# lukebeddow/gripper-mujoco

Measured on AMD Instinct MI355X. Metric: env-steps/sec (batched rollout) at 4096 envs; obs max-rel-err vs C++ ref, higher is better.
Workload: dtype f64; 1 GPU; C3: set6_synthetic 20 mixed objects, randomised spawn (object drawn per episode, spawn_into_scene grid search on the device), steady state: envs staggered over episode steps 1..250 by an untimed pre-roll, benchmark mix (1 episode in 4: the closed-loop grasp-lift-hold program; otherwise the scripted grasp mix: close / squeeze / palm / lift + jitter), canonical sensor/reward config, device auto-rese; envs_per_gpu=4096, global_envs=4096, parallelism=env-shard x1, substeps_per_env_step=63

## Files before the change

__graft_entry__.py:

```python
from __future__ import annotations

import os
import subprocess
import sys

REPO = os.path.dirname(os.path.abspath(__file__))
PKG = os.path.join(REPO, "gripper-mujoco_amd")


def build() -> None:
    if PKG not in sys.path:
        sys.path.insert(0, PKG)
    import threading
    from gmx.build import build as build_lib, build_no_decoupled
    failed = []

    def build_ab():
        try:
            build_no_decoupled()
        except Exception as e:
            failed.append(e)

    ab = threading.Thread(target=build_ab)
    ab.start()
    build_lib(verbose=True)
    ab.join()
    if failed:
        raise failed[0]
    subprocess.run(["make", "-s", "-C", os.path.join(REPO, "oracle"), os.path.join(REPO, "oracle", "liboracle.so")],
                   check=True)
    if os.path.isdir("/root/reference/src"):
        subprocess.run(["make", "-s", "-C", os.path.join(REPO, "oracle"), "ref"], check=True)
    import gmx
    gmx.load_library()


def smoke() -> None:
    import numpy as np
    if PKG not in sys.path:
        sys.path.insert(0, PKG)
    sys.path.insert(0, os.path.join(REPO, "tests"))
    import torch
    assert torch.cuda.is_available(), "smoke() needs a GPU"
    import gmx
    import oracle_lib
    s = gmx.canonical_settings(noise=False, seed=5)
    env = gmx.BatchedGripperEnv(2, object_set="set1_synthetic", settings=s, seed=5, device=0)
    sp = env.make_spawn(x=[0.06, 0.07], y=[0.06, 0.07], idx=0)
    obs0 = env.reset(spawn=sp)
    orc = []
    for e in range(2):
        o = oracle_lib.OracleEnv(env.model, env.cfg, env.objects, e)
        o.reset(sp[e])
        orc.append(o)
        assert np.allclose(obs0[e], o.observation(), atol=1e-5), "reset observation differs from oracle"
    rng = np.random.default_rng(1234)
    for t in range(3):
        a = rng.uniform(-1, 1, size=(2, env.n_actions)).astype(np.float32)
        obs, rew, term, trunc = env.step(a)
        for e in range(2):
            ro, rr, rd = orc[e].step(a[e])
            ro = np.asarray(ro, dtype=np.float64)
            d = np.abs(obs[e] - ro)
            big = np.abs(ro) >= 1e-3
            rel = float((d[big] / np.abs(ro[big])).max()) if big.any() else 0.0
            assert rel <= 1e-4 and float(d[~big].max(initial=0)) <= 1e-4, \
                f"step {t} env {e}: obs rel err {rel:.3e} vs oracle"
            assert bool(term[e]) == bool(rd), "done flag differs from oracle"
            assert abs(float(rew[e]) - float(rr)) <= 1e-5 + 1e-4 * abs(float(rr)), "reward differs from oracle"
    env.close()
    print("smoke ok: 2 envs x 3 env-steps match the oracle")


if __name__ == "__main__":
    build()
    if len(sys.argv) > 1 and sys.argv[1] == "smoke":
        smoke()
```

gripper-mujoco_amd/csrc/gm_capi.hip:

```cpp
#include <hip/hip_runtime.h>

#include <algorithm>
#include <cstddef>
#include <cstdlib>
#include <cstdio>
#include <cmath>
#include <cstring>
#include <map>
#include <string>
#include <vector>
#include <mutex>

#include "gm_kernels.hip"
#include "gm_env_kernels.hip"
#include "gm_policy.hip"
#include "gm_replay.hip"
#include "gm_learn.hip"
#include "gm_ac.hip"
#include "gm_ppo_learn.hip"
#include "gm_sac.hip"
#include "gm_sac_learn.hip"

hipError_t gm_cal_launch_step(int n_seg, int n_envs, hipStream_t st, GmEnvState* states, const gm_model* m,
                              const gm_config* C, const GmTopo* T);
// ... 81 lines not shown

namespace {

int fail(gm_ctx* c, int code, const std::string& msg) {
  if (c) c->err = msg;
  return code;
}
#define HIPCHK(ctx, x)                                                               \
  do {                                                                               \
    hipError_t e_ = (x);                                                             \
    if (e_ != hipSuccess)                                                            \
      return fail(ctx, GM_E_HIP, std::string(#x) + ": " + hipGetErrorString(e_));    \
  } while (0)

static int stage_upload(gm_ctx* c, void* dst, const void* src, size_t bytes) {
  if (bytes <= c->stage_bytes) {
    HIPCHK(c, hipEventSynchronize(c->stage_ev));
    std::memcpy(c->h_stage, src, bytes);
    HIPCHK(c, hipMemcpyAsync(dst, c->h_stage, bytes, hipMemcpyHostToDevice, c->stream));
    HIPCHK(c, hipEventRecord(c->stage_ev, c->stream));
  } else {
    HIPCHK(c, hipMemcpyAsync(dst, src, bytes, hipMemcpyHostToDevice, c->stream));
    HIPCHK(c, hipStreamSynchronize(c->stream));
  }
  return GM_OK;
}
template <class K, class... A>
hipError_t launch_per_env(const gm_ctx* c, K kernel, const A&... args) {
  const int threads = 64, blocks = (c->n_envs + threads - 1) / threads;
  hipLaunchKernelGGL(kernel, dim3(blocks), dim3(threads), 0, c->stream, args...);
  return hipGetLastError();
}
hipError_t upload_mask(gm_ctx* c, const uint8_t* mask, const uint8_t*& dm) {
  dm = mask ? c->d_mask.get() : nullptr;
  return mask ? hipMemcpyAsync(c->d_mask, mask, (size_t)c->n_envs, hipMemcpyHostToDevice, c->stream) : hipSuccess;
}
int read_back(gm_ctx* c, void* dst, const void* src, size_t bytes, int on_device = 0) {
  HIPCHK(c, hipMemcpyAsync(dst, src, bytes, on_device ? hipMemcpyDeviceToDevice : hipMemcpyDeviceToHost, c->stream));
  HIPCHK(c, hipStreamSynchronize(c->stream));
  return GM_OK;
}
hipError_t launch_reset(gm_ctx* c, const uint8_t* dm, const gm_spawn* ds) {
  hipLaunchKernelGGL(gm_reset_kernel, dim3(c->n_envs), dim3(64), 0, c->stream, c->d_state, c->d_model, c->d_cfg,
                     c->d_topo, c->d_eq, dm, ds, c->d_objs, c->n_objects, c->n_envs, c->d_scene, c->scene_tries,
                     c->d_obs, c->spawn_rand);
  return hipGetLastError();
}

bool nseg_supported(int n) {
  switch (n) {
#define X(N) case N:
    GM_NSEG_LIST
#undef X
    return true;
    default: return false;
  }
}
hipError_t launch_step(gm_ctx* c, int grid, int n_envs, int mode, DebugOut dbg, const GmRolloutJob* job = nullptr) {
  const int32_t* order = (mode == 0 && grid == c->n_envs) ? c->d_order.get() : nullptr;
  uint32_t* cost = (mode == 0 && grid == c->n_envs) ? c->d_cost.get() : nullptr;
  const bool chunked = order && c->chunk > 0 && c->chunk_grid > 0 && dbg.phase == nullptr;
  GmChunkQ q{c->d_chunk_ctr, c->d_chunk_ring, c->d_chunk_carry, c->chunk_cap, chunked ? c->chunk : 0,
             c->chunk_margin, c->chunk_yields, c->chunk_cmargin, c->d_chunk_st, c->chunk_steal, c->chunk_prio};
  q.job.steps = 1;
  q.job.driver = GM_DRV_NONE;
  if (job && chunked) q.job = *job;
  if (chunked) grid = c->chunk_grid;
  const bool duo = c->duo && mode == 0;
  switch (c->model.n_seg) {
#define X(N)                                                                                                 \
  case N:                                                                                                    \
    if (duo)                                                                                                 \
      hipLaunchKernelGGL((gm_step_kernel<N + 2, false, true>), dim3(grid), dim3(2 * NT), 0, c->stream,        \
                         c->d_state, c->d_model, c->d_cfg, c->d_topo, c->d_obs, c->d_rew, c->d_done, n_envs,   \
                         mode, dbg, order, cost, q);                                                           \
    else                                                                                                     \
      hipLaunchKernelGGL((gm_step_kernel<N + 2, false>), dim3(grid), dim3(NT), 0, c->stream, c->d_state,      \
                         c->d_model, c->d_cfg, c->d_topo, c->d_obs, c->d_rew, c->d_done, n_envs, mode, dbg,    \
                         order, cost, q);                                                                      \
    return hipGetLastError();
    GM_NSEG_LIST
#undef X
    default: return hipErrorInvalidValue;
  }
}
int timed_launch(gm_ctx* c, const GmRolloutJob* job) {
  DebugOut dbg{nullptr, nullptr, nullptr, nullptr, nullptr};
  HIPCHK(c, hipEventRecord(c->ev0, c->stream));
  HIPCHK(c, launch_step(c, c->n_envs, c->n_envs, 0, dbg, job));
  HIPCHK(c, hipEventRecord(c->ev1, c->stream));
  hipLaunchKernelGGL(gm_dispatch_order_kernel, dim3(1), dim3(1024), 0, c->stream, c->d_cost, c->d_order, c->n_envs,
                     c->d_chunk_ctr, c->d_chunk_st);
  HIPCHK(c, hipGetLastError());
  c->timed = true;
  c->last_launch_steps = job ? job->steps : 1;
  return GM_OK;
}
bool chunk_queue_on(const gm_ctx* c) { return c->chunk > 0 && c->chunk_grid > 0; }
GmRolloutJob rollout_job(const gm_ctx* c, int steps, GmDriver driver, uint64_t seed, float jitter, int max_ep,
                         gm_episode_end* rec) {
  GmRolloutJob j{steps, driver, seed, jitter, max_ep, rec, c->d_eq, c->d_objs, c->n_objects, c->scene_tries,
                 c->d_scene, c->spawn_rand};
  j.sr.env_offset = c->env_offset;
  return j;
}
template <class Before, class After>
int per_step_rollout(gm_ctx* c, int n_steps, int max_ep, gm_episode_end* records, Before before, After after) {
  for (int k = 0; k < n_steps; k++) {
    int rc = before(k);
    if (rc == GM_OK) rc = gm_step(c);
    if (rc == GM_OK) rc = after(k);
    if (rc == GM_OK) rc = gm_autoreset_episodes(c, max_ep, nullptr, 1, nullptr,
                                                records ? records + (size_t)k * c->n_envs : nullptr);
    if (rc != GM_OK) return rc;
  }
  return GM_OK;
}

int build_topo(const gm_model& m, GmTopo& T, std::string& err) {
  std::memset(&T, 0, sizeof(T));
  T.N = m.n_seg;
  T.CL = m.n_seg + 2;
  T.nbody = m.nbody; T.nv = m.nv; T.nq = m.nq; T.ngeom = m.ngeom; T.npair = m.npair; T.nlock = m.nlock;
  T.body_base = m.body_base; T.dof_base = m.dof_base;
  for (int f = 0; f < 3; f++) {
    T.dof_f0[f] = m.dof_pris[f];
    T.body_f0[f] = m.dof_body[m.dof_pris[f]];
    T.body_finger[f] = m.body_finger[f];
  }
  T.body_palm = m.body_palm; T.dof_palm = m.dof_palm;
  T.body_obj = m.body_obj; T.dof_obj = m.dof_obj; T.geom_obj = m.geom_obj;
  T.qadr_obj = m.jnt_qposadr[m.body_jnt[m.body_obj]];
  for (int f = 0; f < 3; f++)
    for (int p = 1; p <= T.CL; p++) {
      int d = T.dof_f0[f] + p - 1, b = T.body_f0[f] + p - 1;
      if (m.dof_body[d] != b || m.body_group[b] != f) { err = "model is not the canonical gripper tree"; return GM_E_ARG; }
      int par = (p == 1) ? m.dof_base : d - 1;
      if (m.dof_parent[d] != par) { err = "unexpected dof parent"; return GM_E_ARG; }
    }
  if (m.npair > GM_MAX_PAIR || m.npair > NT * gm_pair_batches(T.CL) || m.nv > GM_MAX_DOF || T.qadr_obj != m.dof_obj) {
    err = "model exceeds kernel limits";
    return GM_E_RANGE;
  }
  for (int b = 0; b < GM_MAX_BODY; b++) { T.body_group[b] = -1; T.body_cpos[b] = 0; }
  for (int b = 0; b < m.nbody; b++) {
    T.body_group[b] = m.body_group[b];
    if (m.body_group[b] >= 0 && m.body_group[b] < 3) T.body_cpos[b] = b - T.body_f0[m.body_group[b]] + 1;
    else if (m.body_group[b] == GM_GRP_PALM) T.body_cpos[b] = 1;
  }
  for (int l = 0; l < 64; l++) T.lane_body[l] = -1;
  if (T.CL > 15) { err = "finger chain longer than a 16-lane DPP row"; return GM_E_RANGE; }
  for (int f = 0; f < 3; f++)
    for (int p = 1; p <= T.CL; p++) T.lane_body[16 * f + p] = T.body_f0[f] + p - 1;
  T.lane_base = 48;
  T.lane_body[48] = T.body_base;
  T.lane_body[49] = T.body_palm;
  T.lane_body[50] = T.body_obj;
  for (int d = 0; d < m.nv; d++) {
    const int b = m.dof_body[d], j = m.body_jnt[b];
    T.dof_body[d] = b;
    T.dof_grp[d] = m.body_group[b];
    T.dof_p[d] = (m.body_group[b] == GM_GRP_OBJECT) ? d - m.dof_obj : T.body_cpos[b];
    double kp = 0, kd = 0;
    int tgt = 0;
    for (int f = 0; f < 3; f++) {
      if (d == m.dof_pris[f]) { kp = m.kp_gripper[0]; kd = m.kd_gripper[0]; tgt = 1; }
      if (d == m.dof_rev[f]) { kp = m.kp_gripper[1]; kd = m.kd_gripper[1]; tgt = 2; }
    }
    if (d == m.dof_palm) { kp = m.kp_gripper[2]; kd = m.kd_gripper[2]; tgt = 3; }
    if (d == m.dof_base) { kp = m.kp_base[2]; kd = m.kd_base[2]; tgt = 4; }
    const bool free = m.jnt_type[j] == GM_JNT_FREE;
    const bool mj = m.mujoco_actuators != 0;
    double add = m.jnt_armature[j] + (mj ? 0.0 : m.timestep * (m.jnt_damping[j] + kd));
    if (!free && !mj) add += m.timestep * m.timestep * kp;
    T.dof_add[d] = add;
    T.dof_arm[d] = m.jnt_armature[j];
    T.dof_dsum[d] = mj ? 0.0 : m.jnt_damping[j] + kd;
    T.dof_ksum[d] = (free || mj) ? 0.0 : kp;
    T.dof_stiff[d] = free ? 0.0 : m.jnt_stiffness[j];
    T.dof_damp[d] = m.jnt_damping[j];
    T.dof_kp[d] = kp; T.dof_kd[d] = kd; T.dof_target[d] = tgt;
  }
  for (int g = 0; g < m.ngeom; g++) {
    int b = m.geom_body[g];
    T.geom_group[g] = (b == 0) ? -1 : T.body_group[b];
    if (T.geom_group[g] == GM_GRP_BASE) T.geom_group[g] = -1;
    T.geom_cpos[g] = T.body_cpos[b];
  }
  for (int l = 0; l < 64; l++) {
    const int b = T.lane_body[l];
    T.kl_type[l] = -1; T.kl_qadr[l] = 0;
    T.kl_grp[l] = (b >= 0) ? T.body_group[b] : -1;
    const bool chain = T.kl_grp[l] >= 0 && T.kl_grp[l] <= 3;
    T.kl_cpos[l] = chain ? T.body_cpos[b] : 0;
    for (int k = 0; k < 3; k++) { T.kl_pos[l][k] = 0; T.kl_axis[l][k] = 0; }
    T.kl_quat[l][0] = 1; T.kl_quat[l][1] = T.kl_quat[l][2] = T.kl_quat[l][3] = 0;
    if (b > 0) {
      for (int k = 0; k < 3; k++) T.kl_pos[l][k] = m.body_pos[b][k];
      for (int k = 0; k < 4; k++) T.kl_quat[l][k] = m.body_quat[b][k];
      const int j = m.body_jnt[b];
      if (j >= 0) {
        T.kl_type[l] = m.jnt_type[j];
        T.kl_qadr[l] = m.jnt_qposadr[j];
        for (int k = 0; k < 3; k++) T.kl_axis[l][k] = m.jnt_axis[j][k];
      }
    }
  }
  for (int d = 0; d < m.nv; d++) {
    const int j = m.body_jnt[m.dof_body[d]];
    T.dof_jtype[d] = m.jnt_type[j];
    T.dof_k[d] = d - m.jnt_dofadr[j];
    for (int k = 0; k < 3; k++) T.dof_axis[d][k] = m.jnt_axis[j][k];
  }
  for (int p = 0; p < m.npair; p++) {
    const int gs[2] = {m.pair_a[p], m.pair_b[p]};
    for (int s = 0; s < 2; s++) {
      const int g = gs[s];
      T.pr_g[p][s] = g;
      T.pr_type[p][s] = (g == m.geom_obj) ? -1 : m.geom_type[g];
      T.pr_body[p][s] = m.geom_body[g];
      for (int k = 0; k < 3; k++) { T.pr_pos[p][s][k] = m.geom_pos[g][k]; T.pr_size[p][s][k] = m.geom_size[g][k]; }
      for (int k = 0; k < 4; k++) T.pr_quat[p][s][k] = m.geom_quat[g][k];
      T.pr_rbound[p][s] = m.geom_rbound[g];
      T.pr_fric[p][s] = m.geom_friction[g];
    }
  }
  for (int k = 0; k < m.nlock; k++) {
    const int b = m.dof_body[m.lock_dof[k]];
    T.lock_grp[k] = T.body_group[b];
    T.lock_cpos[k] = T.body_cpos[b];
    T.lock_tran[k] = m.body_invweight0[b][0] + m.body_invweight0[m.body_parent[b]][0];
  }
  T.lane_obj = 50;
  T.pair_gobj = -1;
  for (int l = 0; l < 64; l++)
    for (int s = 0; s < 2; s++) { T.lane_opair[l][s] = -1; T.lane_gpair[l][s] = -1; }
  for (int pr = 0; pr < m.npair; pr++) {
    const int a = m.pair_a[pr], bg = m.pair_b[pr];
    const bool with_obj = a == m.geom_obj || bg == m.geom_obj;
    const bool with_gnd = a == m.geom_ground || bg == m.geom_ground;
    if (with_obj && with_gnd) {
      if (T.pair_gobj >= 0) { err = "more than one object-ground pair"; return GM_E_RANGE; }
      T.pair_gobj = pr;
      continue;
    }
    if (!with_obj && !with_gnd) { err = "gripper self-collision pairs are not supported"; return GM_E_RANGE; }
    const int g = with_obj ? (a == m.geom_obj ? bg : a) : (a == m.geom_ground ? bg : a);
    const int b = m.geom_body[g];
    bool assigned = false;
    for (int l = 0; l < 64; l++) {
      if (T.lane_body[l] != b || l == T.lane_obj) continue;
      int32_t* slot = with_obj ? T.lane_opair[l] : T.lane_gpair[l];
      if (slot[0] < 0) slot[0] = pr;
      else if (slot[1] < 0) slot[1] = pr;
      else { err = "a body has more than two object (or ground) pairs"; return GM_E_RANGE; }
      assigned = true;
    }
    if (!assigned) {
      err = "contact pair " + std::to_string(pr) + " is on body " + std::to_string(b) +
            ", which has no scan lane (fingers, palm); the solver cannot take it";
      return GM_E_RANGE;
    }
  }
  return GM_OK;
}

}

namespace {
std::mutex g_settle_mu;
bool g_settle_cache_on = false, g_settle_valid = false;
int g_settle_nseg = -1;
double g_settle_eq[GM_MAX_QPOS];
}

extern "C" {

const char* gm_version(void) { return "gripper-mi355x 0.1 (gfx950, one-wave-per-env fused env-step)"; }

int gm_device_count(void) {
  int n = 0;
  if (hipGetDeviceCount(&n) != hipSuccess) return 0;
  return n;
}

int gm_create(const gm_model* model, const gm_config* cfg, const gm_object* objects, int n_objects,
              int n_envs, int env_offset, int device, uint64_t seed, gm_ctx** out) {
  if (!model || !cfg || !objects || !out || n_envs <= 0 || n_objects <= 0) return GM_E_ARG;
  *out = nullptr;
  gm_ctx* c = new gm_ctx();
  c->device = device;
  c->n_envs = n_envs;
  c->env_offset = env_offset;
  c->n_objects = n_objects;
  c->model = *model;
  c->cfg = *cfg;
  std::string err;
  int rc = build_topo(c->model, c->topo, err);
  if (rc != GM_OK) { fprintf(stderr, "gm_create: %s\n", err.c_str()); delete c; return rc; }
  if (!nseg_supported(c->model.n_seg)) {
    fprintf(stderr, "gm_create: n_seg=%d has no compiled step kernel (GM_NSEG_LIST)\n", c->model.n_seg);
    delete c;
    return GM_E_RANGE;
  }
  {
    const int CLm = c->model.n_seg + 2;
    if (c->model.nbody != 3 * CLm + 4 || c->model.nv != 3 * CLm + 8 || c->model.nq != c->model.nv + 1) {
      fprintf(stderr, "gm_create: model sizes (nbody %d, nv %d, nq %d) do not match the canonical tree for n_seg=%d\n",
              c->model.nbody, c->model.nv, c->model.nq, c->model.n_seg);
      delete c;
// ... 2546 lines not shown
```

gripper-mujoco_amd/csrc/gm_dynamics.h:

```cpp
#pragma once
#include "gm_real.h"
#include "gm_rows.h"

struct Pose { real p[3], q[4], R[9]; };

GM_PHYSICS_BEGIN
template <int CL>
__device__ __forceinline__ void kinematics(SharedT<CL>& S, const gm_model* __restrict__ m, const GmTopo* __restrict__ T, int lane,
                           bool prof = false) {
  unsigned long long t0 = prof ? clock64() : 0;
  real lp[3], lq[4], ax[3] = {0, 0, 0};
  const int b = T->lane_body[lane];
  const int type = T->kl_type[lane];
  ld3(lp, T->kl_pos[lane]);
  ld4(lq, T->kl_quat[lane]);
  if (type >= 0) {
    const real qv = S.s.qpos[T->kl_qadr[lane]];
    ld3(ax, T->kl_axis[lane]);
    if (type == GM_JNT_SLIDE) {
      real R[9], wa[3];
      quat2mat(R, lq);
      mulmv3(wa, R, ax);
      lp[0] += wa[0] * qv; lp[1] += wa[1] * qv; lp[2] += wa[2] * qv;
    } else if (type == GM_JNT_HINGE) {
// ... 93 lines not shown
        cd[0] = cd[1] = cd[2] = 0; cd[3] = cd[4] = cd[5] = 0; cd[3 + k] = 1;
      }
#pragma unroll
      for (int k = 0; k < 3; k++) {
        real* cd = S.cdof[d0 + 3 + k];
        const real w[3] = {R[k], R[3 + k], R[6 + k]};
        cd[0] = w[0]; cd[1] = w[1]; cd[2] = w[2];
        cross3(cd + 3, xp, w);
      }
    } else {
      const int d = chain ? (grp < 3 ? T->dof_f0[grp] + T->kl_cpos[lane] - 1 : T->dof_palm) : T->dof_base;
      real* cd = S.cdof[d];
      real wa[3];
      mulmv3(wa, R, ax);
      if (type == GM_JNT_SLIDE) {
        cd[0] = cd[1] = cd[2] = 0; cd[3] = wa[0]; cd[4] = wa[1]; cd[5] = wa[2];
      } else {
        cd[0] = wa[0]; cd[1] = wa[1]; cd[2] = wa[2];
        cross3(cd + 3, xp, wa);
      }
    }
  }
  GM_WAVE_SYNC();
}

template <int CL>
__device__ __forceinline__ void body_force(SharedT<CL>& S, int b, const real* cvel, const real* cacc) {
  real ci[10], t1[6], t2[6], f[6];
#pragma unroll
  for (int k = 0; k < 10; k++) ci[k] = S.cinert[b][k];
  inert_mul(f, ci, cacc);
  inert_mul(t1, ci, cvel);
  cross_force(t2, cvel, t1);
#pragma unroll
  for (int k = 0; k < 6; k++) S.cfrc[b][k] = f[k] + t2[k];
}
template <int CL>
__device__ __forceinline__ void rne_fwd(SharedT<CL>& S, int b, int d, real* cvel, real* cacc) {
  real cd[6], cdd[6];
#pragma unroll
  for (int k = 0; k < 6; k++) cd[k] = S.cdof[d][k];
  cross_motion(cdd, cvel, cd);
  const real qv = S.s.qvel[d];
#pragma unroll
  for (int k = 0; k < 6; k++) { cvel[k] += cd[k] * qv; cacc[k] += cdd[k] * qv; }
  body_force(S, b, cvel, cacc);
}
template <int L, int CL>
__device__ __forceinline__ void chain_sums(SharedT<CL>& S, int b0, real* fs, real* Is) {
#pragma unroll
  for (int k = 0; k < 6; k++) fs[k] = 0;
#pragma unroll
  for (int k = 0; k < 10; k++) Is[k] = 0;
#pragma unroll
  for (int p = L; p >= 1; p--) {
    const int b = b0 + p - 1;
#pragma unroll
    for (int k = 0; k < 6; k++) { fs[k] += S.cfrc[b][k]; S.cfrc[b][k] = fs[k]; }
#pragma unroll
    for (int k = 0; k < 10; k++) { Is[k] = S.cinert[b][k] + (p < L ? Is[k] : 0.0); S.Ic[b][k] = Is[k]; }
  }
}

template <int CL, bool CAL>
__device__ __forceinline__ void crb_rne(SharedT<CL>& S, const gm_model* __restrict__ m, const GmTopo* __restrict__ T, int lane,
                        bool prof = false) {
  unsigned long long t0 = prof ? clock64() : 0;
  lock_rows<CL, CAL>(S, m, T, lane);
  const int db = T->dof_base;
  const real qdb = S.s.qvel[db];
  real cvb[6], cab[6];
#pragma unroll
  for (int k = 0; k < 6; k++) { cvb[k] = S.cdof[db][k] * qdb; cab[k] = 0; }
  cab[3] = -(real)m->gravity[0]; cab[4] = -(real)m->gravity[1]; cab[5] = -(real)m->gravity[2];

  const int b = T->lane_body[lane];
  const int grp = T->kl_grp[lane];
  const bool chain = grp >= 0 && grp <= 3;
  const int p = T->kl_cpos[lane];
  const int d = chain ? (grp < 3 ? T->dof_f0[grp] + p - 1 : T->dof_palm) : db;
  real cd[6], v[6];
  const real qvd = S.s.qvel[d];
  const real qd = chain ? qvd : 0.0;
#pragma unroll
  for (int k = 0; k < 6; k++) { const real c = S.cdof[d][k]; cd[k] = chain ? c : 0.0; v[k] = cd[k] * qd; }
  real cv[6];
#pragma unroll
  for (int k = 0; k < 6; k++) cv[k] = v[k];
#pragma unroll
  for (int off = 1; off < CL; off <<= 1) {
#pragma unroll
    for (int k = 0; k < 6; k++) {
      const real nb = row_shr(cv[k], off);
      cv[k] += nb;
    }
  }
  real cvp[6];
#pragma unroll
  for (int k = 0; k < 6; k++) {
    const real nb = row_shr(cv[k], 1);
    cvp[k] = cvb[k] + (p > 1 ? nb : 0.0);
    cv[k] += cvb[k];
  }
  real ca[6];
  cross_motion(ca, cvp, cd);
#pragma unroll
  for (int k = 0; k < 6; k++) ca[k] *= qd;
#pragma unroll
  for (int off = 1; off < CL; off <<= 1) {
#pragma unroll
    for (int k = 0; k < 6; k++) {
      const real nb = row_shr(ca[k], off);
      ca[k] += nb;
    }
  }
#pragma unroll
  for (int k = 0; k < 6; k++) ca[k] += cab[k];
  real ci[10], f[6];
#pragma unroll
  for (int k = 0; k < 10; k++) { const real c = S.cinert[b < 0 ? 0 : b][k]; ci[k] = chain ? c : 0.0; }
  {
    real t1[6], t2[6];
    inert_mul(f, ci, ca);
    inert_mul(t1, ci, cv);
    cross_force(t2, cv, t1);
#pragma unroll
    for (int k = 0; k < 6; k++) f[k] += t2[k];
  }
#pragma unroll
  for (int off = 1; off < CL; off <<= 1) {
#pragma unroll
    for (int k = 0; k < 6; k++) {
      const real nb = row_shl(f[k], off);
      f[k] += nb;
    }
#pragma unroll
    for (int k = 0; k < 10; k++) {
      const real nb = row_shl(ci[k], off);
      ci[k] += nb;
    }
  }
  if (chain) {
#pragma unroll
    for (int k = 0; k < 6; k++) S.cfrc[b][k] = f[k];
#pragma unroll
    for (int k = 0; k < 10; k++) S.Ic[b][k] = ci[k];
    if (p == 1) {
#pragma unroll
      for (int k = 0; k < 6; k++) S.chain_f[grp][k] = f[k];
#pragma unroll
      for (int k = 0; k < 10; k++) S.chain_I[grp][k] = ci[k];
    }
  }
  if (b == T->body_obj) {
    const int d0 = T->dof_obj;
    real cvel[6], cacc[6];
#pragma unroll
    for (int k = 0; k < 6; k++) { cvel[k] = 0; cacc[k] = 0; }
    cacc[3] = -(real)m->gravity[0]; cacc[4] = -(real)m->gravity[1]; cacc[5] = -(real)m->gravity[2];
#pragma unroll
    for (int k = 0; k < 3; k++) {
      const real qv = S.s.qvel[d0 + k];
#pragma unroll
      for (int t = 0; t < 6; t++) cvel[t] += S.cdof[d0 + k][t] * qv;
    }
    real cdd[3][6];
#pragma unroll
    for (int k = 0; k < 3; k++) cross_motion(cdd[k], cvel, S.cdof[d0 + 3 + k]);
#pragma unroll
    for (int k = 0; k < 3; k++) {
      const real qv = S.s.qvel[d0 + 3 + k];
#pragma unroll
      for (int t = 0; t < 6; t++) cvel[t] += S.cdof[d0 + 3 + k][t] * qv;
    }
#pragma unroll
    for (int k = 0; k < 3; k++) {
      const real qv = S.s.qvel[d0 + 3 + k];
#pragma unroll
      for (int t = 0; t < 6; t++) cacc[t] += cdd[k][t] * qv;
    }
    body_force(S, b, cvel, cacc);
  }
  GM_WAVE_SYNC();
  PH(17);
  {
    const int bb = T->body_base;
    real ci[10], t1[6], t2[6], fo[6];
#pragma unroll
    for (int k = 0; k < 10; k++) ci[k] = S.cinert[bb][k];
    inert_mul(fo, ci, cab);
    inert_mul(t1, ci, cvb);
    cross_force(t2, cvb, t1);
#pragma unroll
    for (int k = 0; k < 6; k++) fo[k] = fo[k] + t2[k];
    const bool isI = lane < 10;
    const int k = isI ? lane : (lane < 16 ? lane - 10 : 0);
    real own = ci[0];
#pragma unroll
    for (int t = 1; t < 10; t++) own = (lane == t) ? ci[t] : own;
#pragma unroll
    for (int t = 0; t < 6; t++) own = (lane == 10 + t) ? fo[t] : own;
    real acc = own;
#pragma unroll
    for (int c = 0; c < 4; c++) {
      const real vI = S.chain_I[c][k], vf = S.chain_f[c][k];
      acc += isI ? vI : vf;
    }
    if (lane < 16) {
      real* dst = isI ? &S.Ic[bb][k] : &S.cfrc[bb][k];
      *dst = acc;
    }
  }
  GM_WAVE_SYNC();
}

__device__ __forceinline__ void ctrl_gains(const gm_model* __restrict__ m, const GmTopo* __restrict__ T, int d,
                                           real* kp, real* kd) {
  *kp = 0; *kd = 0;
  for (int f = 0; f < 3; f++) {
    if (d == m->dof_pris[f]) { *kp = (real)m->kp_gripper[0]; *kd = (real)m->kd_gripper[0]; }
    if (d == m->dof_rev[f]) { *kp = (real)m->kp_gripper[1]; *kd = (real)m->kd_gripper[1]; }
  }
  if (d == m->dof_palm) { *kp = (real)m->kp_gripper[2]; *kd = (real)m->kd_gripper[2]; }
  if (d == m->dof_base) { *kp = (real)m->kp_base[2]; *kd = (real)m->kd_base[2]; }
}

template <int CL, bool CAL>
__device__ __forceinline__ void mass_and_forces(SharedT<CL>& S, const gm_model* __restrict__ m, const GmTopo* __restrict__ T, int lane) {
  if (lane < T->nv) {
    const int d = lane;
    const int b = T->dof_body[d];
    const int c = T->dof_grp[d];
    const int p = T->dof_p[d];
    real add;
    if constexpr (CAL) {
      const real h = S.s.dt;
      add = T->dof_arm[d] + h * T->dof_dsum[d];
      add += h * h * T->dof_ksum[d];
    } else {
      add = T->dof_add[d];
    }
    real cd[6], F[6];
#pragma unroll
    for (int k = 0; k < 6; k++) cd[k] = S.cdof[d][k];
    inert_mul(F, S.Ic[b], cd);
    if (c == GM_GRP_BASE) {
      S.Hbb = dot6(cd, F) + add;
    } else {
      const bool objd = c == GM_GRP_OBJECT;
      const int d0 = objd ? T->dof_obj : (c < 3) ? T->dof_f0[c] : T->dof_palm;
      real* Hrow = objd ? &S.Ho[TRI(p, 0)] : (c < 3) ? &S.Hf[c][TRI(p, 0)] : &S.Hp[TRI(p, 0)];
#pragma unroll
      for (int q = 0; q <= CL; q++) {
        int dq = objd ? d0 + q : (q == 0) ? T->dof_base : d0 + q - 1;
        dq = dq < SharedT<CL>::NV ? dq : SharedT<CL>::NV - 1;
        real v = dot6(S.cdof[dq], F);
        if (q == p) v += add;
        keep(v);
        if (q <= p) Hrow[q] = v;
      }
    }
    const real bias = dot6(cd, S.cfrc[b]);
    const real qp = S.s.qpos[d], qv = S.s.qvel[d];
    real pas = 0;
    pas -= T->dof_stiff[d] * qp;
    pas -= T->dof_damp[d] * qv;
    const int tgt = T->dof_target[d];
    real act = 0;
    if (tgt != 0) {
      const real target = tgt == 1 ? S.s.next.x : tgt == 2 ? S.s.next.th : tgt == 3 ? S.s.next.z : S.s.base[2];
      act = -((qp - target) * T->dof_kp[d] + qv * T->dof_kd[d]);
    }
    real frc = pas + act - bias;
    if (CAL && S.s.tip_force != 0.0 && (c < 3 || c == GM_GRP_BASE)) {
#pragma unroll
      for (int f = 0; f < 3; f++) {
        if (c < 3 && f != c) continue;
        const int bt = m->body_tip[f];
        real R[9], ip[3], pc[3], wxp[3];
        body_R(S, bt, R);
        ld3(ip, m->body_ipos[bt]);
        mulmv3(pc, R, ip);
        pc[0] += S.xpos[bt][0]; pc[1] += S.xpos[bt][1]; pc[2] += S.xpos[bt][2];
        const real F[3] = {S.s.tip_force * m->tip_dir[f][0], S.s.tip_force * m->tip_dir[f][1],
                           S.s.tip_force * m->tip_dir[f][2]};
        cross3(wxp, cd, pc);
        const real col[3] = {cd[3] + wxp[0], cd[4] + wxp[1], cd[5] + wxp[2]};
        frc += dot3(col, F);
      }
    }
    S.frc[d] = frc;
  }
  GM_WAVE_SYNC();
}
GM_PHYSICS_END
using gmf::kinematics, gmf::crb_rne, gmf::mass_and_forces;
```

gripper-mujoco_amd/csrc/gm_euler.h:

```cpp

#pragma once
#include "gm_arrow.h"

GM_PHYSICS_BEGIN
template <int CL>
__device__ __forceinline__ real euler_factor(const SharedT<CL>& S, const GmTopo* __restrict__ T, real h, int lane,
                                             real (&L)[CL + 1], real& lb, real& invd) {
  const FactorLane fl = factor_lane<CL>(lane);
  const int rowf = fl.rowf, p = fl.p;
  const bool chainrow = fl.chainrow, palm = fl.palm;
  lb = 0.0;
#pragma unroll
  for (int j = 0; j <= CL; j++) L[j] = 0.0;
  if (chainrow) {
    const real* H = S.Hf[rowf];
    const int d = T->dof_f0[rowf] + p - 1;
    const real hd = h * T->dof_damp[d];
    {
      real Hr[CL + 1];
#pragma unroll
      for (int j = 1; j <= CL; j++) Hr[j] = H[j <= p ? TRI(p, j) : TRI(j, p)];
      Hr[0] = Hr[1];
      keep_n<CL + 1>(Hr);
#pragma unroll
      for (int j = 1; j <= CL; j++) L[j] = Hr[j];
    }
#pragma unroll
    for (int j = 1; j <= CL; j++) L[j] = (j == p) ? L[j] + hd : L[j];
    lb = H[TRI(p, 0)];
  } else if (palm) {
    const int d = T->dof_palm;
    const real hd = h * T->dof_damp[d];
    L[1] = S.Hp[TRI(1, 1)] + hd;
    lb = S.Hp[TRI(1, 0)];
  }
  invd = 1.0;
  real ub = 0.0;
  if (lane < 48) {
#pragma unroll
    for (int k = CL; k >= 1; k--) {
      const real ihk = rcp_piv(row_bcast(L[k], k));
      real hk[CL + 1];
#pragma unroll
      for (int j = 1; j < k; j++) hk[j] = row_bcast(L[j], k);
      const real hkb = row_bcast(lb, k);
      const bool upd = p >= 1 && p < k, piv = p == k;
      const real a = L[k] * ihk;
      const real aa = upd ? a : 0.0;
      ub = piv ? lb : ub;
#pragma unroll
      for (int j = 1; j < k; j++) L[j] = L[j] - hk[j] * aa;
      lb = lb - hkb * aa;
      L[k] = upd ? a : L[k];
      invd = piv ? ihk : invd;
    }
#pragma unroll
    for (int j = 1; j < CL; j++) L[j] = (j < p) ? L[j] * invd : L[j];
    lb = lb * invd;
  } else if (palm) {
    const real ih = rcp_piv(L[1]);
    ub = lb;
    lb = lb * ih;
    invd = ih;
  }
  const bool part = chainrow || palm;
  return row_totals(part ? lb * ub : 0.0);
}

template <int CL>
__device__ __forceinline__ void euler_solve(SharedT<CL>& S, const GmTopo* __restrict__ T, real h, int lane,
                                            const real (&L)[CL + 1], real lb, real invd, real sch) {
  const FactorLane fl = factor_lane<CL>(lane);
  const int rowf = fl.rowf, p = fl.p;
  const bool chainrow = fl.chainrow, palm = fl.palm;
  const bool res = S.res_valid != 0;
  real y = 0.0;
  if (chainrow) {
    const int d = T->dof_f0[rowf] + p - 1;
    const real hd = h * T->dof_damp[d];
    y = hd * S.qacc[d];
    if (res) y = y + S.Mv[d];
  } else if (palm) {
    const int d = T->dof_palm;
    const real hd = h * T->dof_damp[d];
    y = hd * S.qacc[d];
    if (res) y = y + S.Mv[d];
  }
  const int db = T->dof_base;
  const real hdb = h * T->dof_damp[db];
  const real bb = S.Hbb + hdb;
  const real yb0 = res ? hdb * S.qacc[db] + S.Mv[db] : hdb * S.qacc[db];
  if (lane < 48) y = chain_forward<CL>(y, L, p);
  const bool part = chainrow || palm;
  const real fs = row_totals(part ? lb * y : 0.0);
  const real xb = (yb0 - fs) * rcp_piv(bb - sch);
  y = y * invd;
  y = y - lb * xb;
  if (lane < 48) y = chain_backward<CL>(y, L, p);
  if (chainrow) {
    const int d = T->dof_f0[rowf] + p - 1;
    S.xs[d] = S.qacc[d] - y;
  } else if (palm) {
    S.xs[T->dof_palm] = S.qacc[T->dof_palm] - y;
  } else if (lane == 48) {
    S.xs[db] = S.qacc[db] - xb;
  } else if (lane >= 57 && lane < 63) {
    const int d = T->dof_obj + lane - 57;
    S.xs[d] = res ? S.qacc[d] - S.Mv[d] : S.qacc[d];
  }
  GM_WAVE_SYNC();
}

template <int CL>
__device__ __forceinline__ void euler_damping(SharedT<CL>& S, const GmTopo* __restrict__ T, real h, int lane) {
  real L[CL + 1], lb, invd;
  const real sch = euler_factor<CL>(S, T, h, lane, L, lb, invd);
  euler_solve<CL>(S, T, h, lane, L, lb, invd, sch);
}
GM_PHYSICS_END
using gmf::euler_factor;
```

gripper-mujoco_amd/csrc/gm_rows.h:

```cpp

#pragma once
#include "gm_real.h"

GM_PHYSICS_BEGIN
__device__ __noinline__ real impedance_pow(real x, real mid, real pw) {
  const bool lo = x <= mid;
  const real t = pow(lo ? x : 1 - x, pw) / pow(lo ? mid : 1 - mid, pw - 1);
  return lo ? t : 1 - t;
}
__device__ __forceinline__ real impedance(const gm_model* __restrict__ m, real r) {
  const real dmin = m->solimp[0], dmax = m->solimp[1], width = m->solimp[2];
  const real mid = m->solimp[3], pw = m->solimp[4];
  if (dmin == dmax || width <= 1e-15) return 0.5 * (dmin + dmax);
  const real x = div_n(fabs(r), width);
  real y;
  if (pw == 2) {
    const bool lo = x <= mid;
    const real q = div_n(lo ? x * x : (1 - x) * (1 - x), lo ? mid : 1 - mid);
    y = lo ? q : 1 - q;
  } else if (pw == 1) {
    y = x;
  } else {
    y = impedance_pow(x, mid, pw);
  }
  real imp = dmin + y * (dmax - dmin);
  imp = (x >= 1) ? dmax : imp;
  imp = (x <= 0) ? dmin : imp;
  return imp;
}

template <int CL, int NVEC>
__device__ void body_vel(SharedT<CL>& S, const real* const* v, real (*const* V)[6], const gm_model* __restrict__ m,
                         const GmTopo* __restrict__ T, int lane, bool obj_only = false) {
  const int db = T->dof_base;
  const int grp = T->kl_grp[lane];
  const bool chain = grp >= 0 && grp <= 3;
  const int p = T->kl_cpos[lane];
  const int d = chain ? (grp < 3 ? T->dof_f0[grp] + p - 1 : T->dof_palm) : db;
  real cvb[NVEC][6], s[NVEC][6];
#pragma unroll
  for (int n = 0; n < NVEC; n++) {
    const real vb = v[n][db];
    const real vd = chain ? v[n][d] : 0.0;
#pragma unroll
    for (int k = 0; k < 6; k++) {
      cvb[n][k] = S.cdof[db][k] * vb;
      const real c = S.cdof[d][k];
      s[n][k] = (chain ? c : 0.0) * vd;
    }
  }
  if (!obj_only) {
#pragma unroll
    for (int off = 1; off < CL; off <<= 1)
#pragma unroll
      for (int n = 0; n < NVEC; n++)
#pragma unroll
        for (int k = 0; k < 6; k++) s[n][k] += row_shr(s[n][k], off);
  }
  const int b = T->lane_body[lane];
  if (chain && !obj_only) {
#pragma unroll
    for (int n = 0; n < NVEC; n++)
#pragma unroll
      for (int k = 0; k < 6; k++) V[n][b][k] = s[n][k] + cvb[n][k];
  } else if (lane == T->lane_base && !obj_only) {
#pragma unroll
    for (int n = 0; n < NVEC; n++)
#pragma unroll
      for (int k = 0; k < 6; k++) V[n][T->body_base][k] = cvb[n][k];
  } else if (b == T->body_obj) {
    const int d0 = T->dof_obj;
    real acc[NVEC][6];
#pragma unroll
    for (int n = 0; n < NVEC; n++)
#pragma unroll
      for (int t = 0; t < 6; t++) acc[n][t] = 0;
#pragma unroll
    for (int k0 = 0; k0 < 6; k0 += 3) {
      real co[18], vk[NVEC][3];
#pragma unroll
      for (int k = 0; k < 3; k++) {
#pragma unroll
        for (int t = 0; t < 6; t++) co[6 * k + t] = S.cdof[d0 + k0 + k][t];
#pragma unroll
        for (int n = 0; n < NVEC; n++) vk[n][k] = v[n][d0 + k0 + k];
      }
      keep_n<18>(co);
#pragma unroll
      for (int k = 0; k < 3; k++)
#pragma unroll
        for (int n = 0; n < NVEC; n++)
#pragma unroll
          for (int t = 0; t < 6; t++) acc[n][t] += co[6 * k + t] * vk[n][k];
    }
#pragma unroll
    for (int n = 0; n < NVEC; n++)
#pragma unroll
      for (int t = 0; t < 6; t++) V[n][b][t] = acc[n][t];
  } else if (lane == 0) {
#pragma unroll
    for (int n = 0; n < NVEC; n++)
#pragma unroll
      for (int k = 0; k < 6; k++) V[n][0][k] = 0.0;
  }
  GM_WAVE_SYNC();
}

template <int CL>
__device__ __forceinline__ void contact_jv(const SharedT<CL>& S, const real (*V)[6], const gm_model* __restrict__ m,
                                           int c, real* jv) {
  const real* C = S.con[c];
  const int b1 = S.cbody[c][0], b2 = S.cbody[c][1];
  const real pos[3] = {C[1], C[2], C[3]};
  real t1v[3], t2v[3];
  cross3(t1v, V[b1], pos);
  cross3(t2v, V[b2], pos);
  const real v1[3] = {V[b1][3] + t1v[0], V[b1][4] + t1v[1], V[b1][5] + t1v[2]};
  const real v2[3] = {V[b2][3] + t2v[0], V[b2][4] + t2v[1], V[b2][5] + t2v[2]};
  const real dv[3] = {v2[0] - v1[0], v2[1] - v1[1], v2[2] - v1[2]};
  const real n[3] = {C[4], C[5], C[6]}, t1[3] = {C[7], C[8], C[9]};
  real t2[3];
  cross3(t2, n, t1);
  const real mu = C[10];
  const real cn = dot3(n, dv), c1 = dot3(t1, dv), c2 = dot3(t2, dv);
  const real m1 = mu * c1, m2 = mu * c2;
  jv[0] = cn + m1; jv[1] = cn - m1; jv[2] = cn + m2; jv[3] = cn - m2;
}
__device__ __forceinline__ void edge_dir(const real* C, const real* t2, int ed, real* u) {
  const real* t = (ed >> 1) ? t2 : C + 7;
  const real mt[3] = {C[10] * t[0], C[10] * t[1], C[10] * t[2]};
  if (ed & 1) { u[0] = C[4] - mt[0]; u[1] = C[5] - mt[1]; u[2] = C[6] - mt[2]; }
  else { u[0] = C[4] + mt[0]; u[1] = C[5] + mt[1]; u[2] = C[6] + mt[2]; }
}

__device__ __forceinline__ real wave_sum(real v) {
#pragma unroll
  for (int s = 32; s >= 1; s >>= 1) v = v + __shfl_xor(v, s);
  return v;
}

struct RowsT {
  real cD, caref[4], cjq[4], cjx[4];
  real lD, laref, ljq, ljx;
  int ldof;
};

template <int CL, bool CAL>
__device__ __forceinline__ void lock_rows(SharedT<CL>& S, const gm_model* __restrict__ m, const GmTopo* __restrict__ T, int lane) {
  const real h = CAL ? S.s.dt : m->timestep;
  real tc = m->solref[0];
  if (tc < 2 * h) tc = 2 * h;
  const real dr = m->solref[1], dmax = m->solimp[1];
  const real K = rcp_n(dmax * dmax * tc * tc * dr * dr);
  const real Bd = div_n(2.0, dmax * tc);
  int nl = 0, k = 0, d = 0;
  real tran = 0.0;
#pragma unroll
  for (int kk = 0; kk < GM_MAX_LOCK; kk++) {
    const bool act = kk < T->nlock && S.s.lock_active[kk];
    const bool mine = act && nl == lane;
    k = mine ? kk : k;
    d = mine ? m->lock_dof[kk] : d;
    tran = mine ? T->lock_tran[kk] : tran;
    nl += act ? 1 : 0;
  }
  {
    const real pos = S.s.qpos[d] - S.s.lock_q[k];
    const real vel = S.s.qvel[d];
    real Da[3], ar[3], av[3];
    bool on[3];
#pragma unroll
    for (int r = 0; r < 3; r++) {
      const real a = S.cdof[d][3 + r];
      av[r] = a;
      on[r] = a != 0.0;
      const real pr = a * pos, vr = a * vel;
      const real imp = impedance(m, pr);
      real Rr = div_n(1 - imp, imp) * tran;
      if (Rr < 1e-15) Rr = 1e-15;
      Da[r] = rcp_n(Rr) * a;
      ar[r] = -Bd * vr - K * imp * pr;
    }
    real De = 0.0, Dar = 0.0;
#pragma unroll
    for (int r = 0; r < 3; r++) {
      De = on[r] ? De + Da[r] * av[r] : De;
      Dar = on[r] ? Dar + Da[r] * ar[r] : Dar;
    }
    const int slot = lane < nl ? lane : GM_MAX_LOCK;
    S.lrow_D[slot] = De;
    S.lrow_aref[slot] = div_n(Dar, De);
    S.lrow_dof[slot] = d;
  }
  S.nl = nl;
}

template <int CL, bool CAL>
__device__ __forceinline__ void contact_rows(SharedT<CL>& S, const gm_model* __restrict__ m, const GmTopo* __restrict__ T,
                                             int lane, real (*V)[6], real (*V2)[6], real& cD, real* caref, real* jq,
                                             bool& obj_only) {
  const real h = CAL ? S.s.dt : m->timestep;
  real tc = m->solref[0];
  if (tc < 2 * h) tc = 2 * h;
  const real dr = m->solref[1], dmax = m->solimp[1];
  const real K = rcp_n(dmax * dmax * tc * tc * dr * dr);
  const real Bd = div_n(2.0, dmax * tc);
  {
    const real* vv[2] = {S.s.qvel, S.s.qacc_warm};
    real (*VV[2])[6] = {V, V2};
    bool og = true;
    if (lane < S.ncon) {
      const int b1 = S.cbody[lane][0], b2 = S.cbody[lane][1];
      og = (b1 == 0 && b2 == T->body_obj) || (b2 == 0 && b1 == T->body_obj);
    }
    obj_only = __ballot(!og) == 0ull;
    body_vel<CL, 2>(S, vv, VV, m, T, lane, obj_only);
  }
#pragma unroll
  for (int e = 0; e < 4; e++) jq[e] = 0.0;
  cD = 0;
#pragma unroll
  for (int e = 0; e < 4; e++) caref[e] = 0;
  if (lane < S.ncon) {
    const real* C = S.con[lane];
    const int b1 = S.cbody[lane][0], b2 = S.cbody[lane][1];
    const real oiw = S.s.obj_invw[0], biw1 = m->body_invweight0[b1][0], biw2 = m->body_invweight0[b2][0];
    const real iw1 = (b1 == T->body_obj) ? oiw : biw1;
    const real iw2 = (b2 == T->body_obj) ? oiw : biw2;
    const real tran = iw1 + iw2;
    const real mu = C[10];
    const real diag = tran + (mu * mu) * tran;
    const real imp = impedance(m, C[0]);
    real Rr = div_n(1 - imp, imp) * diag;
    if (Rr < 1e-15) Rr = 1e-15;
    cD = rcp_n(Rr);
    real vel[4], jv[4];
    contact_jv<CL>(S, V, m, lane, vel);
    contact_jv<CL>(S, V2, m, lane, jv);
#pragma unroll
    for (int e = 0; e < 4; e++) {
      caref[e] = -Bd * vel[e] - K * imp * C[0];
      jq[e] = jv[e] - caref[e];
    }
  }
}

template <int CL>
struct DuoRows {
  real cD[GM_MAX_CON], caref[4][GM_MAX_CON], jq[4][GM_MAX_CON];
  int32_t obj_only;
};
// ... 66 lines not shown
```

gripper-mujoco_amd/csrc/gm_shared.h:

```cpp
#pragma once
#include <hip/hip_runtime.h>
#include <stdint.h>
#include "gm_state.h"
#include "gm_math.h"

#define NT 64
#define GM_WAVE_SYNC() do { __builtin_amdgcn_fence(__ATOMIC_SEQ_CST, "wavefront"); \
                            __builtin_amdgcn_wave_barrier(); } while (0)
#define GM_ENV_SYNC() do { __builtin_amdgcn_fence(__ATOMIC_RELEASE, "workgroup"); \
                           __builtin_amdgcn_wave_barrier(); \
                           __builtin_amdgcn_fence(__ATOMIC_ACQUIRE, "workgroup"); } while (0)
__device__ __forceinline__ int fresh_lane() {
  int lane;
  asm volatile("v_mbcnt_lo_u32_b32 %0, -1, 0\n\tv_mbcnt_hi_u32_b32 %0, -1, %0" : "=v"(lane));
  return lane;
}
__device__ __forceinline__ void keep(double x) { asm volatile("" ::"v"(x)); }
template <int N>
__device__ __forceinline__ void keep_n(const double* a) {
  static_assert(N >= 1 && N <= 28, "keep_n: 1..28 values");
#define GM_K(i) "v"(a[(i) < N ? (i) : 0])
  if constexpr (N <= 13) {
    asm volatile("" ::GM_K(0), GM_K(1), GM_K(2), GM_K(3), GM_K(4), GM_K(5), GM_K(6), GM_K(7), GM_K(8), GM_K(9),
                 GM_K(10), GM_K(11), GM_K(12));
  } else {
    asm volatile("" ::GM_K(0), GM_K(1), GM_K(2), GM_K(3), GM_K(4), GM_K(5), GM_K(6), GM_K(7), GM_K(8), GM_K(9),
                 GM_K(10), GM_K(11), GM_K(12), GM_K(13), GM_K(14), GM_K(15), GM_K(16), GM_K(17), GM_K(18),
                 GM_K(19), GM_K(20), GM_K(21), GM_K(22), GM_K(23), GM_K(24), GM_K(25), GM_K(26), GM_K(27));
  }
#undef GM_K
}
#define GM_BB_SLOTS 18
#ifndef GM_NSEG_LIST
#define GM_NSEG_LIST X(5) X(6) X(7) X(8) X(9) X(10)
#endif
#define CLMAX (GM_MAX_SEG + 2)
#define TRI(p, q) ((p) * ((p) + 1) / 2 + (q))
#define TRIF ((CLMAX + 1) * (CLMAX + 2) / 2)
#define CW (CL + 8)
#define PI_F 3.14159265358979f

typedef double real;
#define GM_EPI_ATTR __device__

struct DebugOut {
  int32_t* ncon;
  double* contact;
  double* efc_force;
  double* qacc;
  unsigned long long* phase;
  int32_t* nefc;
  double* wrench;
};
#define GM_NPHASE 32

template <int CL>
struct __align__(16) SharedT {
  static constexpr int NB = 3 * CL + 4;
  static constexpr int NV = 3 * CL + 8;
  static constexpr int TRIC = (CL + 1) * (CL + 2) / 2;
  GmEnvHot s;
  real lock_pre[GM_MAX_LOCK];
  real lrow_D[GM_MAX_LOCK + 1], lrow_aref[GM_MAX_LOCK + 1];
  int32_t lrow_dof[GM_MAX_LOCK + 2];
  real qacc[NV];
  real xs[NV];
  real Ma[NV], Mv[NV];
  real xpos[NB][3];
  real xquat[NB][4];
  real Hf[3][TRIC], Hp[3], Ho[21], Hbb;
  real cdof[NV][6];
  real frc[NV];
  real go[27];
  real con[GM_MAX_CON][14];
  int16_t cgeom[GM_MAX_CON][2];
  int16_t cbody[GM_MAX_CON][2];
  int16_t pair_off[GM_MAX_PAIR], pair_cnt[GM_MAX_PAIR];
  union {
    struct {
      union {
        real cinert[NB][10];
        real Ic[NB][10];
      };
      real cfrc[NB][6];
      real chain_f[5][6], chain_I[5][10];
    };
    struct { real QF[GM_MAX_CON][9]; real V[NB][6]; } nw;
    struct { real V[NB][6]; real V2[NB][6]; } nw2;
    struct { real qf_[GM_MAX_CON][9]; real root[4][54]; real comp[54]; real oo[27]; } st;
    struct { real lbub[3][CL][14]; real plb[14]; real bbx[28]; real ych[3][CL]; real ypalm; } fs;
    struct { real efc[GM_MAX_EFC]; } dbg;
    struct { real hit[GM_BB_SLOTS][8][4]; } cl;
  };
  static_assert(sizeof(real[GM_BB_SLOTS][8][4]) <= sizeof(real) * (GM_MAX_CON * 9 + 4 * 54 + 54 + 27),
                "box-box hit slots must fit inside the chain-root stage (st): they may not grow the union");
  int32_t ncon, nefc, nl, overflow;
  int32_t res_valid;
  int32_t duo_cmd;
  int32_t work_nefc, work_mpr, work_newton;
  int32_t stp_fixed;
  float forces[32];
  int32_t have_forces;
  float gauge_tmp[3];
  int32_t bend_ready;
  double next_read;
  unsigned long long tph[GM_NPHASE];
  GmEnvState* gs;
};

#define PH(k) do { MARK(k); if (__builtin_expect(prof, 0)) { unsigned long long t_ = clock64(); if (lane == 0) S.tph[k] += t_ - t0; t0 = t_; } } while (0)
#ifdef GM_ISA_MARKERS
#define MARK(k) asm volatile("s_nop 15\n\ts_nop " #k)
#else
#define MARK(k) do { } while (0)
#endif
```

gripper-mujoco_amd/gmx/build.py:

```python
from __future__ import annotations

import os
import subprocess

from ._lib import PKG_DIR, REPO_DIR, LIB_PATH

SOURCES = ["csrc/gm_capi.hip", "csrc/gm_calib.hip", "csrc/gm_host_model.cpp", "csrc/gm_mjcf.cpp"]
HIPCC = os.environ.get("HIPCC", "/opt/rocm/bin/hipcc")
FLAGS = ["--offload-arch=gfx950", "-O3", "-std=c++17", "-fPIC",
         "-fhip-fp32-correctly-rounded-divide-sqrt", "-munsafe-fp-atomics",
         "-ffp-contract=off",
         "-mllvm", "-disable-machine-licm"]


NO_DECOUPLED_LIB = os.path.join(os.path.dirname(LIB_PATH), "libgm_no_decoupled.so")


def _deps():
    csrc = os.path.join(PKG_DIR, "csrc")
    return sorted(os.path.join(PKG_DIR, s) for s in SOURCES) + \
        sorted(os.path.join(csrc, f) for f in os.listdir(csrc) if f.endswith((".hip", ".h", ".inc"))) + \
        [os.path.join(REPO_DIR, "include", f) for f in ("gripper_mi355x.h", "gm_settings.def")]


def build_no_decoupled(verbose: bool = False) -> str:
    if os.path.exists(NO_DECOUPLED_LIB):
        t = os.path.getmtime(NO_DECOUPLED_LIB)
        if all(os.path.getmtime(d) <= t for d in _deps()):
            return NO_DECOUPLED_LIB
    return build(verbose=verbose, out=NO_DECOUPLED_LIB, extra_flags=["-DGM_NO_DECOUPLED_POINT"])


def build(verbose: bool = False, force: bool = False, out: str | None = None, extra_flags=()) -> str:
    lib_path = out or LIB_PATH
    srcs = [os.path.join(PKG_DIR, s) for s in SOURCES]
    csrc = os.path.join(PKG_DIR, "csrc")
    deps = sorted(set(srcs + [os.path.join(csrc, f) for f in os.listdir(csrc) if f.endswith((".hip", ".h", ".inc"))])) + \
        [os.path.join(REPO_DIR, "include", f) for f in ("gripper_mi355x.h", "gm_settings.def")]
    if not force and out is None and os.path.exists(LIB_PATH):
        t = os.path.getmtime(LIB_PATH)
        if all(os.path.getmtime(d) <= t for d in deps):
            return LIB_PATH
    objdir = os.path.join(os.path.dirname(LIB_PATH), "obj" if out is None else "obj_" + os.path.basename(out))
    os.makedirs(objdir, exist_ok=True)
    inc = ["-I" + os.path.join(REPO_DIR, "include"), "-I" + os.path.join(PKG_DIR, "csrc")]
    procs, objs = [], []
    headers = [os.path.join(csrc, "gm_state.h")] + \
        [os.path.join(REPO_DIR, "include", f) for f in ("gripper_mi355x.h", "gm_settings.def")]
    for src in srcs:
        obj = os.path.join(objdir, os.path.basename(src) + ".o")
        objs.append(obj)
        tu_deps = [src] + headers if src.endswith(".cpp") else deps
        if not force and os.path.exists(obj) and all(os.path.getmtime(d) <= os.path.getmtime(obj) for d in tu_deps):
            continue
        cmd = [HIPCC, *FLAGS, *extra_flags, *inc, "-c", src, "-o", obj]
        if verbose:
            print(" ".join(cmd))
        procs.append((subprocess.Popen(cmd), cmd))
    for p, cmd in procs:
        if p.wait() != 0:
            raise subprocess.CalledProcessError(p.returncode, cmd)
    link = [HIPCC, "--offload-arch=gfx950", "-shared", "-fPIC", *objs, "-o", lib_path + ".tmp"]
    if verbose:
        print(" ".join(link))
    subprocess.run(link, check=True)
    os.replace(lib_path + ".tmp", lib_path)
    return lib_path
```

Baseline: 774,400 env-steps/s.

## Spread object free-joint velocity and bias work across six component lanes

The object body's cvel/cacc computation and the per-vector motion transform used to run serially on one lane. They are now split across six dedicated lanes (57–62), one per spatial component, and the results are gathered with readlane and a shared-memory exchange. This is meant to shorten that single-lane critical path inside the wavefront's dynamics pass. In exchange it adds a wave sync, shared scratch writes and several cross-lane reads. A compile flag keeps the old path for A/B builds, and a new check rejects layouts where a body's scan lane would overlap those lanes.

```diff
diff --git a/__graft_entry__.py b/__graft_entry__.py
--- a/__graft_entry__.py
+++ b/__graft_entry__.py
@@ -12,12 +12,13 @@
     if PKG not in sys.path:
         sys.path.insert(0, PKG)
     import threading
-    from gmx.build import build as build_lib, build_no_decoupled
+    from gmx.build import build as build_lib, build_no_decoupled, build_no_object_lanes
     failed = []
 
     def build_ab():
         try:
             build_no_decoupled()
+            build_no_object_lanes()
         except Exception as e:
             failed.append(e)
 
diff --git a/gripper-mujoco_amd/csrc/gm_capi.hip b/gripper-mujoco_amd/csrc/gm_capi.hip
--- a/gripper-mujoco_amd/csrc/gm_capi.hip
+++ b/gripper-mujoco_amd/csrc/gm_capi.hip
@@ -257,10 +257,12 @@
   if (T.CL > 15) { err = "finger chain longer than a 16-lane DPP row"; return GM_E_RANGE; }
   for (int f = 0; f < 3; f++)
     for (int p = 1; p <= T.CL; p++) T.lane_body[16 * f + p] = T.body_f0[f] + p - 1;
-  T.lane_base = 48;
-  T.lane_body[48] = T.body_base;
-  T.lane_body[49] = T.body_palm;
-  T.lane_body[50] = T.body_obj;
+  T.lane_base = GM_LANE_BASE;
+  T.lane_body[GM_LANE_BASE] = T.body_base;
+  T.lane_body[GM_LANE_BASE + 1] = T.body_palm;
+  T.lane_body[GM_LANE_BASE + 2] = T.body_obj;
+  for (int l = GM_OBJ_LANE0; l < GM_OBJ_LANE0 + 6; l++)
+    if (T.lane_body[l] >= 0) { err = "a body's scan lane on the object's component lanes"; return GM_E_RANGE; }
   for (int d = 0; d < m.nv; d++) {
     const int b = m.dof_body[d], j = m.body_jnt[b];
     T.dof_body[d] = b;
diff --git a/gripper-mujoco_amd/csrc/gm_dynamics.h b/gripper-mujoco_amd/csrc/gm_dynamics.h
--- a/gripper-mujoco_amd/csrc/gm_dynamics.h
+++ b/gripper-mujoco_amd/csrc/gm_dynamics.h
@@ -269,6 +269,43 @@
       for (int k = 0; k < 10; k++) S.chain_I[grp][k] = ci[k];
     }
   }
+#ifndef GM_NO_OBJECT_LANES
+  {
+    const int d0 = T->dof_obj;
+    const int ol = lane - GM_OBJ_LANE0;
+    const int t = ol < 0 ? 0 : (ol > 5 ? 5 : ol);
+    const int kr = t < 3 ? t : 2;
+    real qv[6], cdt[6], cdk[6];
+#pragma unroll
+    for (int k = 0; k < 6; k++) { qv[k] = S.s.qvel[d0 + k]; cdt[k] = S.cdof[d0 + k][t]; cdk[k] = S.cdof[d0 + 3 + kr][k]; }
+    real cvt = 0;
+#pragma unroll
+    for (int k = 0; k < 3; k++) cvt += cdt[k] * qv[k];
+    real cw[6], cdd[6];
+#pragma unroll
+    for (int k = 0; k < 6; k++) cw[k] = readlane_real(cvt, GM_OBJ_LANE0 + k);
+    cross_motion(cdd, cw, cdk);
+    if (ol >= 0 && ol < 3) {
+#pragma unroll
+      for (int k = 0; k < 6; k++) S.go[6 * ol + k] = cdd[k];
+    }
+#pragma unroll
+    for (int k = 0; k < 3; k++) cvt += cdt[3 + k] * qv[3 + k];
+    GM_WAVE_SYNC();
+    real cat = 0;
+#pragma unroll
+    for (int k = 0; k < 3; k++) cat = (t == 3 + k) ? -(real)m->gravity[k] : cat;
+#pragma unroll
+    for (int k = 0; k < 3; k++) cat += S.go[6 * k + t] * qv[3 + k];
+    real cvel[6], cacc[6];
+#pragma unroll
+    for (int k = 0; k < 6; k++) {
+      cvel[k] = readlane_real(cvt, GM_OBJ_LANE0 + k);
+      cacc[k] = readlane_real(cat, GM_OBJ_LANE0 + k);
+    }
+    if (b == T->body_obj) body_force(S, b, cvel, cacc);
+  }
+#else
   if (b == T->body_obj) {
     const int d0 = T->dof_obj;
     real cvel[6], cacc[6];
@@ -298,6 +335,7 @@
     }
     body_force(S, b, cvel, cacc);
   }
+#endif
   GM_WAVE_SYNC();
   PH(17);
   {
diff --git a/gripper-mujoco_amd/csrc/gm_euler.h b/gripper-mujoco_amd/csrc/gm_euler.h
--- a/gripper-mujoco_amd/csrc/gm_euler.h
+++ b/gripper-mujoco_amd/csrc/gm_euler.h
@@ -104,8 +104,8 @@
     S.xs[T->dof_palm] = S.qacc[T->dof_palm] - y;
   } else if (lane == 48) {
     S.xs[db] = S.qacc[db] - xb;
-  } else if (lane >= 57 && lane < 63) {
-    const int d = T->dof_obj + lane - 57;
+  } else if (lane >= GM_OBJ_LANE0 && lane < GM_OBJ_LANE0 + 6) {
+    const int d = T->dof_obj + lane - GM_OBJ_LANE0;
     S.xs[d] = res ? S.qacc[d] - S.Mv[d] : S.qacc[d];
   }
   GM_WAVE_SYNC();
diff --git a/gripper-mujoco_amd/csrc/gm_rows.h b/gripper-mujoco_amd/csrc/gm_rows.h
--- a/gripper-mujoco_amd/csrc/gm_rows.h
+++ b/gripper-mujoco_amd/csrc/gm_rows.h
@@ -68,6 +68,26 @@
     for (int n = 0; n < NVEC; n++)
 #pragma unroll
       for (int k = 0; k < 6; k++) V[n][T->body_base][k] = cvb[n][k];
+#ifndef GM_NO_OBJECT_LANES
+  } else if (lane >= GM_OBJ_LANE0 && lane < GM_OBJ_LANE0 + 6) {
+    const int d0 = T->dof_obj, t = lane - GM_OBJ_LANE0;
+    real co[6], vk[NVEC][6], acc[NVEC];
+#pragma unroll
+    for (int k = 0; k < 6; k++) {
+      co[k] = S.cdof[d0 + k][t];
+#pragma unroll
+      for (int n = 0; n < NVEC; n++) vk[n][k] = v[n][d0 + k];
+    }
+    keep_n<6>(co);
+#pragma unroll
+    for (int n = 0; n < NVEC; n++) acc[n] = 0;
+#pragma unroll
+    for (int k = 0; k < 6; k++)
+#pragma unroll
+      for (int n = 0; n < NVEC; n++) acc[n] += co[k] * vk[n][k];
+#pragma unroll
+    for (int n = 0; n < NVEC; n++) V[n][T->body_obj][t] = acc[n];
+#else
   } else if (b == T->body_obj) {
     const int d0 = T->dof_obj;
     real acc[NVEC][6];
@@ -97,6 +117,7 @@
     for (int n = 0; n < NVEC; n++)
 #pragma unroll
       for (int t = 0; t < 6; t++) V[n][b][t] = acc[n][t];
+#endif
   } else if (lane == 0) {
 #pragma unroll
     for (int n = 0; n < NVEC; n++)
diff --git a/gripper-mujoco_amd/csrc/gm_shared.h b/gripper-mujoco_amd/csrc/gm_shared.h
--- a/gripper-mujoco_amd/csrc/gm_shared.h
+++ b/gripper-mujoco_amd/csrc/gm_shared.h
@@ -39,6 +39,10 @@
 #define TRIF ((CLMAX + 1) * (CLMAX + 2) / 2)
 #define CW (CL + 8)
 #define PI_F 3.14159265358979f
+#define GM_LANE_BASE 48
+#define GM_OBJ_LANE0 57
+static_assert(32 + CLMAX < GM_LANE_BASE && GM_LANE_BASE + 2 < GM_OBJ_LANE0 && GM_OBJ_LANE0 + 6 <= 64,
+              "the object's component lanes must hold no body's scan lane");
 
 typedef double real;
 #define GM_EPI_ATTR __device__
diff --git a/gripper-mujoco_amd/gmx/build.py b/gripper-mujoco_amd/gmx/build.py
--- a/gripper-mujoco_amd/gmx/build.py
+++ b/gripper-mujoco_amd/gmx/build.py
@@ -23,12 +23,23 @@
         [os.path.join(REPO_DIR, "include", f) for f in ("gripper_mi355x.h", "gm_settings.def")]
 
 
+def _build_variant(lib: str, flag: str, verbose: bool) -> str:
+    if os.path.exists(lib):
+        t = os.path.getmtime(lib)
+        if all(os.path.getmtime(d) <= t for d in _deps()):
+            return lib
+    return build(verbose=verbose, out=lib, extra_flags=[flag])
+
+
 def build_no_decoupled(verbose: bool = False) -> str:
-    if os.path.exists(NO_DECOUPLED_LIB):
-        t = os.path.getmtime(NO_DECOUPLED_LIB)
-        if all(os.path.getmtime(d) <= t for d in _deps()):
-            return NO_DECOUPLED_LIB
-    return build(verbose=verbose, out=NO_DECOUPLED_LIB, extra_flags=["-DGM_NO_DECOUPLED_POINT"])
+    return _build_variant(NO_DECOUPLED_LIB, "-DGM_NO_DECOUPLED_POINT", verbose)
+
+
+NO_OBJECT_LANES_LIB = os.path.join(os.path.dirname(LIB_PATH), "libgm_no_object_lanes.so")
+
+
+def build_no_object_lanes(verbose: bool = False) -> str:
+    return _build_variant(NO_OBJECT_LANES_LIB, "-DGM_NO_OBJECT_LANES", verbose)
 
 
 def build(verbose: bool = False, force: bool = False, out: str | None = None, extra_flags=()) -> str:
```

Result: faster. 791,100 env-steps/s (median of 6 runs) (+2.2%).
